# samivout/clair-torch

Measured on AMD Instinct MI355X. Metric: MPix/s HDR-merged (+uncertainty) at N=32 4K RGB, higher is better.
Workload: dtype f32; 1 GPU; C2: 32-exposure 4096x4096x3 uint16 stack per GPU, merge+uncertainty (LINEAR ICRF 3x256, Gaussian weights, sigma: multiplier, float64 mean + float32 std out); global_image=4096x4096x3 in 1 row band(s)

## Files before the change

### clair_torch_amd/csrc/ct_merge.hip

```cpp
#include "ct_merge.hpp"
#include <type_traits>

#ifndef CT_MERGE_PART
#define CT_MERGE_PART 0
#endif

namespace ct {

template <typename T, int V, int INTERP, int WEIGHT, int STD, bool FOLD, int PF = 2, bool PIVOT = true>
__global__ __launch_bounds__(kBlock) void merge_kernel(const MergeArgs a)
{
    extern __shared__ __align__(16) char lds[];
    constexpr bool kInt = sizeof(T) != 4;
    constexpr bool kRanged = kInt;
    constexpr bool kHasStd = STD != CT_STD_NONE;
    constexpr bool kGauss = WEIGHT == CT_WEIGHT_GAUSS;
    constexpr int kEntry = lut_entry_bytes(INTERP);
    static_assert(!FOLD || kInt, "FOLD is for integer codes");
    using Moment = std::conditional_t<PIVOT, float, double>;
    const int C = a.channels, L = a.n_points, B = a.batch;
    const int lut_bytes = INTERP == CT_INTERP_NONE ? 0 : C * L * kEntry;
    float *inv_t = reinterpret_cast<float *>(lds + lut_bytes);
    float *cq = inv_t + B;
    const float top = INTERP == CT_INTERP_NONE ? 1.0f : (float)(L - 1);
// ... 368 lines not shown
        __builtin_amdgcn_make_buffer_rsrc(reinterpret_cast<void *>(base), 0, 0xffffffff, 0x00020000 );
    P out;
    if constexpr (sizeof(P) == 1) {
        const uint8_t v = __builtin_amdgcn_raw_buffer_load_b8(rsrc, offset, 0, CT_STACK_LOAD_AUX);
        __builtin_memcpy(&out, &v, sizeof(P));
    } else if constexpr (sizeof(P) == 2) {
        const uint16_t v = __builtin_amdgcn_raw_buffer_load_b16(rsrc, offset, 0, CT_STACK_LOAD_AUX);
        __builtin_memcpy(&out, &v, sizeof(P));
    } else if constexpr (sizeof(P) == 4) {
        const uint32_t v = __builtin_amdgcn_raw_buffer_load_b32(rsrc, offset, 0, CT_STACK_LOAD_AUX);
        __builtin_memcpy(&out, &v, sizeof(P));
    } else if constexpr (sizeof(P) == 8) {
        typedef uint32_t vec_t __attribute__((ext_vector_type(2)));
        const vec_t v = __builtin_amdgcn_raw_buffer_load_b64(rsrc, offset, 0, CT_STACK_LOAD_AUX);
        __builtin_memcpy(&out, &v, sizeof(P));
    } else {
        static_assert(sizeof(P) == 16, "packets are at most 16 bytes");
        typedef uint32_t vec_t __attribute__((ext_vector_type(4)));
        const vec_t v = __builtin_amdgcn_raw_buffer_load_b128(rsrc, offset, 0, CT_STACK_LOAD_AUX);
        __builtin_memcpy(&out, &v, sizeof(P));
    }
    return out;
}

#ifndef CT_PIVOT_TYPED_LOAD
#define CT_PIVOT_TYPED_LOAD 1
#endif
template <typename T, int V>
__device__ __forceinline__ Packet<float, V> load_codes_as_float(uint64_t base, uint32_t offset)
{
    Packet<float, V> out;
    load_codes_as_float<T, V, CT_STACK_LOAD_AUX>(base, offset, out.v);
    return out;
}


template <int N, int I = 0, typename F>
__device__ __forceinline__ void static_for(F &&f)
{
    if constexpr (I < N) {
        f(std::integral_constant<int, I>{});
        static_for<N, I + 1>(f);
    }
}

struct PivotArgs {
    uint32_t index_mul;
    float step;
    uint32_t n_tiles;
    int32_t probe;
    float index_rcp;
    float max_code;
    float tf_max;
    uint32_t n_entries;
    unsigned long long *retry_count;
    int32_t n_batches;
    int32_t fresh;
    int32_t batch_size[16];
    const void *batch_ptr[16];
    const float *std_ptr[16];
    int32_t rgb252;
    uint32_t stage_off;
};
constexpr int kMaxMultiBatches = 16;
constexpr int kPivotV = 4;

#ifndef CT_PIVOT_DEPTH
#define CT_PIVOT_DEPTH 2
#endif
constexpr int kPivotDepth = CT_PIVOT_DEPTH;
constexpr float kRoughLimit = 64.0f;

#ifndef CT_PIVOT_WEIGHT
#define CT_PIVOT_WEIGHT 0
#endif
#ifndef CT_PIVOT_WT_SHIFT
#define CT_PIVOT_WT_SHIFT 4
#endif

#ifndef CT_RGB252_WAVES
#define CT_RGB252_WAVES 6
#endif
#ifndef CT_PIVOT_KERNEL_ATTR
#define CT_PIVOT_KERNEL_ATTR __attribute__((amdgpu_waves_per_eu(FIRST && V <= 4 && STD != CT_STD_EXPLICIT ? (CT_PIVOT_TYPED_LOAD ? (RGB252 ? CT_RGB252_WAVES : 7) : 8) : 4, 8)))
#endif
template <typename T, int V, int INTERP, int WEIGHT, int STD, bool FIRST, bool CLAMP = false, bool MULTI = false, bool RGB252 = false>
__global__ __launch_bounds__(kBlock) CT_PIVOT_KERNEL_ATTR void merge_pivot_kernel(const MergeArgs a, const PivotArgs x)
{
    static_assert(!MULTI || (!FIRST && CT_PIVOT_TYPED_LOAD), "MULTI carries state and uses the typed loads");
    static_assert(!RGB252 || (V == 4 && FIRST && !MULTI && CT_PIVOT_TYPED_LOAD), "RGB252: single-batch packets of the typed-load kernel");
    extern __shared__ __align__(16) char lds[];
    static_assert(sizeof(T) != 4, "raw integer codes only");
    static_assert(CT_PIVOT_TYPED_LOAD || ((INTERP == CT_INTERP_LINEAR || INTERP == CT_INTERP_NONE) && !CLAMP), "raw-load build: whole-step LINEAR only");
    constexpr bool kLut = INTERP != CT_INTERP_NONE;
    constexpr bool kLookup = INTERP == CT_INTERP_LOOKUP;
    constexpr bool kCat = INTERP == CT_INTERP_CATMULL;
    constexpr bool kHasStd = STD != CT_STD_NONE;
    constexpr bool kGauss = WEIGHT == CT_WEIGHT_GAUSS;
    constexpr bool kTyped = CT_PIVOT_TYPED_LOAD;
    using CodePk = std::conditional_t<kTyped, Packet<float, V>, Packet<T, V>>;
    const int C = a.channels, L = a.n_points, B = a.batch;
    constexpr int kWV = (INTERP == CT_INTERP_LINEAR && kGauss && kTyped && sizeof(T) == 2 && V == 4) ? CT_PIVOT_WEIGHT : 0;
    constexpr int kEntryShift = (kWV == 2 || kCat) ? 4 : 3;
    const int E = kLut ? (int)x.n_entries : 0;
    const int lut_bytes = C * E * (1 << kEntryShift);
    float2 *expo = reinterpret_cast<float2 *>(lds + lut_bytes);
    [[maybe_unused]] const uint32_t wt_base = (uint32_t)lut_bytes + 8u * (uint32_t)B;
    const float kk = sqrtf(a.weight_scale * 1.4426950408889634f);
    const float dk_mul = kk * a.inv_max_code, dk_add = -0.5f * kk;
    const float K = -2.0f * a.weight_scale;
    const float max_code = kLut ? x.max_code : 1.0f;
    const float ce = kGauss ? max_code * kk / K : max_code;

    bool rough = false;
    if constexpr (kLookup) {
        const int total = C * E;
        for (int k = threadIdx.x; k < total; k += kBlock) {
            const int r = k / E, j = k - r * E;
            const int idx = (j + 1) >> 1;
            reinterpret_cast<float2 *>(lds)[k] = make_float2(a.lut[(size_t)r * L + (idx < L ? idx : L - 1)], 0.0f);
        }
    } else if constexpr (kCat) {
        const int total = C * L;
        const double st = (double)x.step;
        for (int k = threadIdx.x; k < total; k += kBlock) {
            const int r = k / L, i = k - r * L;
            const float *row = a.lut + (size_t)r * L;
            const double p0 = row[i > 0 ? i - 1 : 0], p1 = row[i], p2 = row[i + 1 < L ? i + 1 : L - 1], p3 = row[i + 2 < L ? i + 2 : L - 1];
            const double c1 = 0.5 * (p2 - p0), b1 = 0.5 * (2.0 * p0 - 5.0 * p1 + 4.0 * p2 - p3), a1 = 0.5 * (-p0 + 3.0 * p1 - 3.0 * p2 + p3);
            reinterpret_cast<float4 *>(lds)[k] = make_float4((float)p1, (float)(c1 / st), (float)(b1 / (st * st)), (float)(a1 / (st * st * st)));
        }
    } else if constexpr (kLut) {
        const int total = C * L;
        const double stepd = (double)x.max_code / (double)(L - 1);
        bool viol = false;
        for (int k = threadIdx.x; k < total; k += kBlock) {
            const int r = k / L, i = k - r * L;
            const float *row = a.lut + (size_t)r * L;
            const float g0 = row[i], g1 = row[i + 1 < L ? i + 1 : L - 1];
            const float slope = (g1 - g0) / x.step;
            const float A = (float)((double)g0 - (double)slope * ((double)i * stepd));
            viol |= !(fabsf(A) <= kRoughLimit * fmaxf(fmaxf(fabsf(g0), fabsf(g1)), 1e-30f));
        }
        rough = __syncthreads_or(viol);
        for (int k = threadIdx.x; k < total; k += kBlock) {
            const int r = k / L, i = k - r * L;
            const float *row = a.lut + (size_t)r * L;
            const float g0 = row[i], g1 = row[i + 1 < L ? i + 1 : L - 1];
            const float slope = (g1 - g0) / x.step;
            const float A = (float)((double)g0 - (double)slope * ((double)i * stepd));
            if constexpr (kWV == 2) {
                const double dki = (double)i * (double)x.step * (double)dk_mul + (double)dk_add;
                reinterpret_cast<float4 *>(lds)[k] =
                    make_float4(rough ? g0 : A, slope, (float)exp2(-dki * dki), (float)(-2.0 * dki * (double)dk_mul));
            } else {
                reinterpret_cast<float2 *>(lds)[k] = make_float2(rough ? g0 : A, slope);
            }
        }
    }
    if constexpr (kWV == 1) {
        constexpr int s = CT_PIVOT_WT_SHIFT, nW = 65536 >> s;
        for (int j = threadIdx.x; j < nW; j += kBlock) {
            const double c0 = (double)(j << s), c1 = (double)((j + 1) << s);
            const double d0 = c0 * (double)dk_mul + (double)dk_add, d1 = c1 * (double)dk_mul + (double)dk_add;
            const double w0 = exp2(-d0 * d0), w1 = exp2(-d1 * d1), ws = (w1 - w0) / (c1 - c0);
            *reinterpret_cast<float2 *>(lds + wt_base + 8u * (uint32_t)j) = make_float2((float)(w0 - ws * c0), (float)ws);
        }
    }
    for (int n = threadIdx.x; n < B; n += kBlock) {
        const float it = (float)(1.0 / a.exposure[n]);
        expo[n] = make_float2(it, ce * it);
    }
    __syncthreads();

    const bool finalize = a.flags & CT_MERGE_FINALIZE;
    const bool keep_state = a.mean_state != nullptr;
    const bool planar = a.tile.layout == CT_LAYOUT_NCHW;
    const bool planar_out = planar || (a.flags & CT_MERGE_OUT_AS_INPUT);
    float fsf = 1.0f;
    if constexpr (kGauss) fsf = K / kk;
    if constexpr (STD == CT_STD_CONSTANT) fsf *= a.std_value;
    if constexpr (STD == CT_STD_MULTIPLIER) fsf *= a.std_value * a.inv_max_code;
    const float sv2 = fsf * fsf;
    [[maybe_unused]] const uint32_t index_mul = x.index_mul & 0xffffffu;
    [[maybe_unused]] const float index_rcp = x.index_rcp;
    [[maybe_unused]] float floor_magic = kFloorMagic;
    asm volatile("" : "+v"(floor_magic));

    constexpr bool rgb252 = RGB252;
    for (uint32_t tile = blockIdx.x; tile < x.n_tiles; tile += gridDim.x) {
        const uint32_t vec = tile * (uint32_t)kBlock + threadIdx.x;
        if (vec * (uint32_t)V >= a.q_count) continue;
        const uint32_t q0 = a.q_begin + vec * (uint32_t)V;

        int row_off[V];
        if constexpr (kLut) {
            if (planar) {
                int ch = 0;
                for (int c = 1; c < C; ++c) ch += q0 >= (uint32_t)c * a.tile.plane_local ? 1 : 0;
                const uint32_t qg = q0 + (uint32_t)ch * a.tile.chan_skip + a.tile.base;
                uint32_t off = q0 - (uint32_t)ch * a.tile.plane_local;
                int r = C == 3 ? (int)(qg % 3u) : (int)(qg % (uint32_t)C);
                const int skip_mod = (int)(a.tile.chan_skip % (uint32_t)C);
#pragma unroll
                for (int e = 0; e < V; ++e) {
                    row_off[e] = (kLookup ? ch : r) * E * 8;
                    int inc = 1;
                    if (++off == a.tile.plane_local) {
                        off = 0;
                        ++ch;
                        inc += skip_mod;
                    }
                    r += inc;
                    r = r >= C ? r - C : r;
                }
            } else if (C == 3) {
                const uint32_t plane_g = a.tile.plane_local + a.tile.chan_skip;
#pragma unroll
                for (int e = 0; e < V; ++e) {
                    uint32_t c, pixel;
                    a.tile.interleaved3(q0 + e, c, pixel);
                    const uint32_t qg = c * plane_g + a.tile.base + pixel;
                    row_off[e] = (int)(kLookup ? c : qg % 3u) * E * 8;
                }
            } else {
#pragma unroll
                for (int e = 0; e < V; ++e) {
                    int ch;
                    uint32_t qg;
                    a.tile.locate(a.tile.planar_index(q0 + e), ch, qg);
                    row_off[e] = (kLookup ? ch : (int)(qg % (uint32_t)C)) * E * 8;
                }
            }
        } else {
#pragma unroll
            for (int e = 0; e < V; ++e) row_off[e] = 0;
        }
        [[maybe_unused]] uint32_t rowc[V];
        if constexpr (kTyped && kLut) {
#pragma unroll
            for (int e = 0; e < V; ++e) rowc[e] = lds_row_constant<kEntryShift>(row_off[e] << (kEntryShift - 3));
        }

        const uint32_t voff = q0 * (uint32_t)sizeof(T), svoff = q0 * 4u;
        auto planar_of = [&](uint32_t m) -> uint32_t {
            if (planar_out) return m;
            if (C == 3) {
                uint32_t c, pixel;
                a.tile.interleaved3(m, c, pixel);
                return c * a.tile.plane_local + pixel;
            }
            return a.tile.planar_index(m);
        };

        constexpr int VS = FIRST ? 1 : V;
        float p[V], WA[VS], varA[VS];
        double meanA[VS];
        [[maybe_unused]] auto probe_pivot = [&](uint64_t stack_base) {
            const Packet<float, V> pk = load_codes_as_float<T, V>(
                stack_base + (uint64_t)((int64_t)x.probe * a.image_stride * (int64_t)sizeof(T)), voff);
            const float itp = expo[x.probe].x;
            float tf[V];
            if constexpr (kLut) floor_index_bits<V>(pk.v, index_rcp, floor_magic, tf);
            if constexpr (kLut && CLAMP) {
#pragma unroll
                for (int e = 0; e < V; ++e) tf[e] = fminf(tf[e], x.tf_max);
            }
#pragma unroll
            for (int e = 0; e < V; ++e) {
                const float px = pk.v[e];
                float lin = px * a.inv_max_code;
                if constexpr (kCat) {
                    const float4 g = *reinterpret_cast<const float4 *>(lds + lds_entry_address<kEntryShift>(tf[e], rowc[e]));
                    float o = __builtin_fmaf(tf[e] - floor_magic, -x.step, px);
                    if constexpr (CLAMP) o = px > x.max_code ? 0.0f : o;
                    lin = __builtin_fmaf(__builtin_fmaf(__builtin_fmaf(g.w, o, g.z), o, g.y), o, g.x);
                } else if constexpr (kLut) {
                    const float2 g = *reinterpret_cast<const float2 *>(lds + lds_entry_address<kEntryShift>(tf[e], rowc[e]));
                    lin = __builtin_fmaf(g.y, rough ? __builtin_fmaf(tf[e] - floor_magic, -x.step, px) : px, g.x);
                }
                p[e] = lin * itp;
            }
        };
        if constexpr (FIRST && kTyped) {
            probe_pivot(reinterpret_cast<uint64_t>(a.stack));
        } else if constexpr (FIRST) {
            const Packet<T, V> pk = load_buffer<Packet<T, V>>(
                reinterpret_cast<uint64_t>(a.stack) + (uint64_t)((int64_t)x.probe * a.image_stride * (int64_t)sizeof(T)), voff);
            const float itp = expo[x.probe].x;
            static_for<V>([&](auto ec) {
                constexpr int e = decltype(ec)::value;
                float lin = code_to_float<T, V, e>(pk) * a.inv_max_code;
                if constexpr (kLut) {
                    const uint32_t i0 = code_to_interval<T, V, e>(pk, index_mul);
                    const float2 g = *reinterpret_cast<const float2 *>(lds + (row_off[e] + (int)(i0 << 3)));
                    const float px = code_to_float<T, V, e>(pk);
                    lin = __builtin_fmaf(g.y, rough ? __builtin_fmaf((float)i0, -x.step, px) : px, g.x);
                }
                p[e] = lin * itp;
            });
        } else {
            bool fresh = false;
            if constexpr (MULTI) fresh = x.fresh != 0;
            if (fresh) {
                if constexpr (MULTI) {
#pragma unroll
                    for (int e = 0; e < V; ++e) {
                        meanA[e] = 0.0;
                        WA[e] = 0.0f;
                        varA[e] = 0.0f;
                    }
                    probe_pivot(reinterpret_cast<uint64_t>(x.batch_ptr[0]));
                }
            } else {
#pragma unroll
                for (int e = 0; e < V; ++e) {
                    const uint32_t q = planar_of(q0 + e);
                    meanA[e] = a.mean_state[q];
                    WA[e] = a.sumw_state[q];
                    if constexpr (kHasStd) varA[e] = a.var_state[q];
                    p[e] = (float)meanA[e];
                }
            }
        }

        double mean_o[V];
        float var_o[V], Wt_o[V];
        const int n_batches = MULTI ? x.n_batches : 1;
        int n0 = 0;
        for (int bi = 0; bi < n_batches; ++bi) {
        const int Bb = MULTI ? x.batch_size[bi] : B;
        const uint64_t batch_base = MULTI ? reinterpret_cast<uint64_t>(x.batch_ptr[bi]) : reinterpret_cast<uint64_t>(a.stack);
        [[maybe_unused]] const uint64_t batch_std_base = MULTI ? reinterpret_cast<uint64_t>(x.std_ptr[bi]) : reinterpret_cast<uint64_t>(a.std_stack);
        for (int pass = 0;; ++pass) {
            float W[V], Swy[V], Saa[V], Sac[V], Scc[V];
#pragma unroll
            for (int e = 0; e < V; ++e) W[e] = Swy[e] = Saa[e] = Sac[e] = Scc[e] = 0.0f;

            auto run_batch = [&](auto rough_c, auto moments_c) {
            constexpr bool kRough = decltype(rough_c)::value;
            constexpr bool kMoments = decltype(moments_c)::value;
            auto reduce = [&](const CodePk &pk, const Packet<float, V> &sp, uint32_t expo_adr) {
                const float2 ex = *reinterpret_cast<const float2 *>(lds + expo_adr);
                const float it = ex.x, cqn = ex.y;
                float pxv[V], ga[V], gs[V];
                [[maybe_unused]] float pxl[V];
                [[maybe_unused]] float dkv[V], wv[V];
                [[maybe_unused]] float tf[V], tw[V], gw[V], gd[V];
                if constexpr (kTyped) {
#pragma unroll
                    for (int e = 0; e < V; ++e) pxv[e] = pk.v[e];
                    if constexpr (kLut && kWV == 1)
                        floor_index_bits2<V>(pxv, index_rcp, 1.0f / (float)(1 << CT_PIVOT_WT_SHIFT), floor_magic, tf, tw);
                    else if constexpr (kLut)
                        floor_index_bits<V>(pxv, index_rcp, floor_magic, tf);
                    if constexpr (kLut && CLAMP) {
#pragma unroll
                        for (int e = 0; e < V; ++e) tf[e] = fminf(tf[e], x.tf_max);
                    }
                }
                static_for<V>([&](auto ec) {
                    constexpr int e = decltype(ec)::value;
                    if constexpr (kTyped) {
                        if constexpr (kLut && kWV == 2) {
                            float4 g = *reinterpret_cast<const float4 *>(lds + lds_entry_address<4>(tf[e], rowc[e]));
                            asm volatile("" : "+v"(g.x), "+v"(g.y), "+v"(g.z), "+v"(g.w));
                            ga[e] = g.x;
                            gs[e] = g.y;
                            gw[e] = g.z;
                            gd[e] = g.w;
                            pxl[e] = __builtin_fmaf(tf[e] - floor_magic, -x.step, pxv[e]);
                        } else if constexpr (kCat) {
                            const float4 g = *reinterpret_cast<const float4 *>(lds + lds_entry_address<4>(tf[e], rowc[e]));
                            float o = __builtin_fmaf(tf[e] - floor_magic, -x.step, pxv[e]);
                            [[maybe_unused]] bool above = false;
                            if constexpr (CLAMP) {
                                above = pxv[e] > x.max_code;
                                o = above ? 0.0f : o;
                            }
                            ga[e] = __builtin_fmaf(__builtin_fmaf(__builtin_fmaf(g.w, o, g.z), o, g.y), o, g.x);
                            gs[e] = 0.0f;
                            if constexpr (kHasStd) {
                                gs[e] = __builtin_fmaf(__builtin_fmaf(3.0f * g.w, o, g.z + g.z), o, g.y);
                                if constexpr (CLAMP) gs[e] = above ? 0.0f : gs[e];
                            }
                        } else if constexpr (kLut) {
                            const float2 g = *reinterpret_cast<const float2 *>(lds + lds_entry_address(tf[e], rowc[e]));
                            ga[e] = g.x;
                            gs[e] = g.y;
                            if constexpr (kRough) pxl[e] = __builtin_fmaf(tf[e] - floor_magic, -x.step, pxv[e]);
                            if constexpr (kWV == 1) {
                                const float2 wt = *reinterpret_cast<const float2 *>(
                                    lds + lds_entry_address(tw[e], wt_base - (kFloorMagicBits << 3)));
                                gw[e] = wt.x;
                                gd[e] = wt.y;
                            }
                        }
                    } else {
                    pxv[e] = code_to_float<T, V, e>(pk);
                    if constexpr (kLut) {
                        const uint32_t i0 = code_to_interval<T, V, e>(pk, index_mul);
                        const float2 g = *reinterpret_cast<const float2 *>(lds + (row_off[e] + (int)(i0 << 3)));
                        ga[e] = g.x;
                        gs[e] = g.y;
                        if constexpr (kRough) pxl[e] = __builtin_fmaf((float)i0, -x.step, pxv[e]);
                    }
                    }
                    if constexpr (kGauss) {
                        dkv[e] = __builtin_fmaf(pxv[e], dk_mul, dk_add);
                        if constexpr (kWV == 0) wv[e] = __builtin_amdgcn_exp2f(-dkv[e] * dkv[e]);
                    }
                });
                if constexpr (kWV == 1) {
#pragma unroll
                    for (int e = 0; e < V; ++e) wv[e] = __builtin_fmaf(gd[e], pxv[e], gw[e]);
                }
                if constexpr (kWV == 2) {
                    const float m2 = dk_mul * dk_mul;
#pragma unroll
                    for (int e = 0; e < V; ++e) {
                        const float v = pxl[e] * __builtin_fmaf(pxl[e], -m2, gd[e]);
                        float q = __builtin_fmaf(v, 0.009618129107628477f, 0.05550410866482158f);
                        q = __builtin_fmaf(q, v, 0.2402265069591007f);
                        q = __builtin_fmaf(q, v, 0.6931471805599453f);
                        q = __builtin_fmaf(q, v, 1.0f);
                        wv[e] = gw[e] * q;
                    }
                }
                if constexpr (kGauss && kWV == 0) {
#pragma unroll
                    for (int e = 0; e < V; ++e) asm volatile("" : "+v"(wv[e]));
                }
#pragma unroll
                for (int e = 0; e < V; ++e) {
                    const float px = pxv[e];
                    const float lin = (kLookup || kCat) ? ga[e] : kLut ? __builtin_fmaf(gs[e], kRough ? pxl[e] : px, ga[e]) : px * a.inv_max_code;
                    const float yd = __builtin_fmaf(lin, it, -p[e]);
                    if constexpr (kGauss) {
                        const float dk = dkv[e], w = wv[e];
                        W[e] += w;
                        Swy[e] = __builtin_fmaf(w, yd, Swy[e]);
                        if constexpr (kHasStd && kMoments) {
                            float wu = w;
                            if constexpr (STD == CT_STD_MULTIPLIER) wu = w * px;
                            if constexpr (STD == CT_STD_EXPLICIT) wu = w * sp.v[e];
                            const float av = dk * wu;
                            float cv;
                            if constexpr (kLookup) {
                                cv = av * yd;
                            } else {
                                const float ev = kLut ? (wu * gs[e]) * cqn : wu * cqn;
                                cv = __builtin_fmaf(av, yd, ev);
                            }
                            Saa[e] = __builtin_fmaf(av, av, Saa[e]);
                            Sac[e] = __builtin_fmaf(av, cv, Sac[e]);
                            Scc[e] = __builtin_fmaf(cv, cv, Scc[e]);
                        }
                    } else {
                        Swy[e] += yd;
                        if constexpr (kHasStd) {
                            float ev = kLut ? gs[e] * cqn : cqn;
                            if constexpr (STD == CT_STD_MULTIPLIER) ev *= px;
                            if constexpr (STD == CT_STD_EXPLICIT) ev *= sp.v[e];
                            Scc[e] = __builtin_fmaf(ev, ev, Scc[e]);
                        }
                    }
                }
            };

            auto fetch = [&](int n, CodePk &pk, Packet<float, V> &sp) {
                const int nn = n < Bb ? n : Bb - 1;
                uint64_t base = batch_base + (uint64_t)((int64_t)nn * a.image_stride * (int64_t)sizeof(T));
                asm volatile("" : "+s"(base));
                if constexpr (kTyped)
                    pk = load_codes_as_float<T, V>(base, voff);
                else
                    pk = load_buffer<Packet<T, V>>(base, voff);
                if constexpr (STD == CT_STD_EXPLICIT) {
                    uint64_t sbase = batch_std_base + (uint64_t)((int64_t)nn * a.image_stride * 4);
                    asm volatile("" : "+s"(sbase));
                    sp = load_buffer<Packet<float, V>>(sbase, svoff);
                }
            };
            constexpr int kRing = kPivotDepth + 1;
            CodePk ring[kRing];
            Packet<float, V> sring[STD == CT_STD_EXPLICIT ? kRing : 1];
            static_for<kPivotDepth>([&](auto jc) {
                constexpr int j = decltype(jc)::value;
                fetch(j, ring[j], sring[STD == CT_STD_EXPLICIT ? j : 0]);
            });
            uint32_t expo_adr = (uint32_t)lut_bytes + 8u * (uint32_t)n0;
            for (int n = 0; n < Bb; n += kRing) {
                static_for<kRing>([&](auto jc) {
                    constexpr int j = decltype(jc)::value, slot = (j + kPivotDepth) % kRing;
                    fetch(n + j + kPivotDepth, ring[slot], sring[STD == CT_STD_EXPLICIT ? slot : 0]);
                    if (j == 0 || n + j < Bb) reduce(ring[j], sring[STD == CT_STD_EXPLICIT ? j : 0], expo_adr + 8u * j);
                });
                expo_adr += 8u * kRing;
            }
            };
            constexpr bool kMeanFirst = kLookup && kHasStd;
            if constexpr (kMeanFirst) {
                if (pass == 0)
                    run_batch(std::false_type{}, std::false_type{});
                else
                    run_batch(std::false_type{}, std::true_type{});
            } else {
                if (rough)
                    run_batch(std::true_type{}, std::true_type{});
                else
                    run_batch(std::false_type{}, std::true_type{});
            }

            bool bad[V];
            float mb_f[V];
#pragma unroll
            for (int e = 0; e < V; ++e) {
                const float Wb = kGauss ? W[e] : (float)Bb;
                const float Df = Wb + 1e-6f;
                const float r = __builtin_amdgcn_rcpf(Df);
                const float num = __builtin_fmaf(-p[e], 1e-6f, Swy[e]);
                float q = num * r;
                q = __builtin_fmaf(__builtin_fmaf(-q, Df, num), r, q);
                float Wt = Wb, frac = 1.0f, var = 0.0f, gam = 0.0f;
                bad[e] = false;
                if constexpr (FIRST) {
                    mean_o[e] = (double)p[e] + (double)q;
                } else {
                    Wt = WA[e] + Wb;
                    const float rw = __builtin_amdgcn_rcpf(Wt);
                    frac = WA[e] == 0.0f ? 1.0f : Wb * rw;
                    const double diff = ((double)p[e] - meanA[e]) + (double)q;
                    mean_o[e] = __builtin_fma((double)frac, diff, meanA[e]);
                    gam = ((WA[e] * rw) * rw) * (float)diff;
                    var = varA[e];
                }
                Wt_o[e] = Wt;
                mb_f[e] = p[e] + q;
                if constexpr (kHasStd) {
                    const float beta = frac * r;
                    const float kap = __builtin_fmaf(-beta, q, gam);
                    const float bk = beta * kap;
                    const float S = __builtin_fmaf(kap * kap, Saa[e], (beta * beta) * Scc[e]);
                    const float upd = __builtin_fmaf(bk + bk, Sac[e], S);
                    if constexpr (kGauss) bad[e] = upd * (0.5f * (kPivotCondLimit + 1.0f)) < S;
                    if constexpr (kMeanFirst) bad[e] = bad[e] || pass == 0;
                    var += fmaxf(upd, 0.0f) * sv2;
                }
                var_o[e] = var;
            }
            bool any_bad = false;
#pragma unroll
            for (int e = 0; e < V; ++e) any_bad |= bad[e];
            if (pass == 1 || !__any(any_bad)) break;
            if (x.retry_count && (threadIdx.x & 63) == 0) atomicAdd(x.retry_count, 1ull);
#pragma unroll
            for (int e = 0; e < V; ++e) p[e] = bad[e] ? mb_f[e] : p[e];
        }
        if constexpr (MULTI) {
#pragma unroll
            for (int e = 0; e < V; ++e) {
                meanA[e] = mean_o[e];
                WA[e] = Wt_o[e];
                varA[e] = var_o[e];
                p[e] = (float)mean_o[e];
            }
            n0 += Bb;
        }
        }

        if (keep_state) {
#pragma unroll
            for (int e = 0; e < V; ++e) {
                const uint32_t q = planar_of(q0 + e);
                a.mean_state[q] = mean_o[e];
                a.sumw_state[q] = Wt_o[e];
                if constexpr (kHasStd) a.var_state[q] = var_o[e];
            }
        }
        if (finalize && rgb252) {
            if constexpr (RGB252) {
                const uint32_t tile_first = tile * (uint32_t)(kBlock * V);
// ... 354 lines not shown
        }
    }
    if (q_vec) {
        a.q_begin = 0;
        a.q_count = q_vec;
        rc = dispatch_interp<T, V>(a, interp, weight_mode, std_mode, s, fold);
        if (rc != CT_OK) return rc;
    }
    if (q_vec < Q) {
        a.q_begin = q_vec;
        a.q_count = Q - q_vec;
        rc = dispatch_interp<T, 1>(a, interp, weight_mode, std_mode, s, fold);
    }
    return rc;
}

#endif

}

#if CT_MERGE_PART != 1

extern "C" int ct_norm_constants(float max_code, float *hi, float *lo);
extern "C" int ct_index_constants(float max_code, int n_points, float *hi, float *lo);
extern "C" int ct_pivot_index_constants(float max_code, int n_points, uint32_t *index_mul, float *step);
extern "C" int ct_pivot_floor_constants(float max_code, int n_points, float *rcp_step);

static unsigned long long *g_merge_retry_counter = nullptr;
extern "C" void ct_merge_set_retry_counter(unsigned long long *counter_dev) { g_merge_retry_counter = counter_dev; }

extern "C" int ct_pivot_interval_constants(float max_code, int n_points, int lookup, int dtype_max, float *scale);

static bool pivot_eligible(int32_t dtype, float max_code, int interp, int n_points, uint32_t flags, ct::PivotArgs *px,
                           bool *clamp = nullptr)
{
    if (dtype != CT_DTYPE_U8 && dtype != CT_DTYPE_U16) return false;
    const int dtype_max = dtype == CT_DTYPE_U8 ? 255 : 65535;
    if (flags & CT_MERGE_F64_MOMENTS) return false;
    if (!(max_code >= 1.0f) || max_code > (float)dtype_max || floorf(max_code) != max_code) return false;
    if (interp < CT_INTERP_LOOKUP || interp > CT_INTERP_NONE) return false;
    if (interp == CT_INTERP_CATMULL && !CT_PIVOT_TYPED_LOAD) return false;
    const bool need_clamp = interp != CT_INTERP_NONE && max_code < (float)dtype_max;
    if (clamp) *clamp = need_clamp;
    px->step = 1.0f;
    px->index_mul = 0;
    px->index_rcp = 1.0f;
    px->max_code = max_code;
    px->n_entries = 0;
    px->tf_max = ct::kFloorMagic;
    if (interp == CT_INTERP_NONE) return true;
    if (CT_PIVOT_TYPED_LOAD) {
        if (need_clamp && dtype == CT_DTYPE_U8) return false;
        const bool lookup = interp == CT_INTERP_LOOKUP;
        if (ct_pivot_interval_constants(max_code, n_points, lookup, dtype_max, &px->index_rcp) != CT_OK) return false;
        px->step = (float)((double)max_code / (double)(n_points - 1));
        px->n_entries = lookup ? 2u * (uint32_t)n_points : (uint32_t)n_points;
        px->tf_max = ct::kFloorMagic + (float)(lookup ? 2 * (n_points - 1) : n_points - 1);
        return true;
    }
    if (interp != CT_INTERP_LINEAR || need_clamp) return false;
    if (ct_pivot_index_constants(max_code, n_points, &px->index_mul, &px->step) != CT_OK) return false;
    if (dtype == CT_DTYPE_U8 && px->step != 1.0f) return false;
    if (dtype == CT_DTYPE_U16 && px->index_mul == 0) return false;
    px->n_entries = (uint32_t)n_points;
    return true;
}

static bool merge_uses_reference_order(int interp, int std_mode, uint32_t flags)
{
    if (flags & CT_MERGE_REFERENCE_ORDER) return true;
    return (interp == CT_INTERP_CATMULL || interp == CT_INTERP_LOOKUP) && std_mode != CT_STD_NONE &&
           !(flags & (CT_MERGE_CLOSED_FORM | CT_MERGE_F64_MOMENTS));
}

extern "C" const char *ct_hdr_merge_kernel_name(int32_t dtype, float max_code, int32_t interp, int32_t n_points,
                                                uint32_t flags)
{
    if (merge_uses_reference_order(interp, (flags & CT_MERGE_STD_HINT) ? CT_STD_CONSTANT : CT_STD_NONE, flags))
        return "ct::merge_reference_order_kernel (the reference's float32 autograd order, two passes, float64 exp and divisions)";
    ct::PivotArgs px{};
    if (pivot_eligible(dtype, max_code, interp, interp == CT_INTERP_NONE ? 2 : n_points, flags, &px))
        return (flags & CT_MERGE_FIRST_BATCH)
                   ? "ct::merge_pivot_kernel (float32 moments about a per-pixel pivot, persistent workgroups, 4 codes per "
                     "thread through typed buffer loads, 7 wavefronts per SIMD, first batch)"
                   : "ct::merge_pivot_kernel (float32 moments about the running mean, persistent workgroups, 4 codes per "
                     "thread, streaming state)";
    if (flags & CT_MERGE_F64_MOMENTS)
        return dtype == CT_DTYPE_F32 ? "ct::merge_kernel (float64 moments, float32 pixels, 4 per thread)"
                                     : "ct::merge_kernel (float64 moments, integer codes)";
    return dtype == CT_DTYPE_F32 ? "ct::merge_kernel (float32 moments about a per-pixel pivot, float32 pixels, 4 per thread)"
                                 : "ct::merge_kernel (float32 moments about a per-pixel pivot, integer codes through the float LUT coordinate)";
}

extern "C" int ct_hdr_merge_batch(const void *stack_dev, int32_t dtype, float max_code, int32_t batch,
                                  const ct_geometry *geom, const float *std_dev, int32_t std_mode, float std_value,
                                  const double *exposure_dev, const ct_icrf *icrf, int32_t weight_mode,
                                  double *mean_state_dev, float *sumw_state_dev, float *var_state_dev,
                                  void *mean_out_dev, float *std_out_dev, uint32_t flags, void *stream)
{
    using namespace ct;
    if (!stack_dev || !geom || !icrf || !exposure_dev || batch <= 0) return CT_ERR_INVALID_ARGUMENT;
    if (geom->channels <= 0 || geom->h_tile <= 0 || geom->width <= 0 || geom->h_global < geom->h_tile ||
        geom->row_offset < 0 || geom->row_offset + geom->h_tile > geom->h_global)
        return CT_ERR_INVALID_ARGUMENT;
    if (geom->layout < CT_LAYOUT_NCHW || geom->layout > CT_LAYOUT_NHWC_BGR) return CT_ERR_INVALID_ARGUMENT;
    const int interp = icrf->interp;
    if (interp < CT_INTERP_LOOKUP || interp > CT_INTERP_NONE) return CT_ERR_INVALID_ARGUMENT;
    if (interp != CT_INTERP_NONE && (!icrf->lut_dev || icrf->n_points < 2)) return CT_ERR_INVALID_ARGUMENT;
    if (std_mode < CT_STD_NONE || std_mode > CT_STD_EXPLICIT) return CT_ERR_INVALID_ARGUMENT;
    if (std_mode == CT_STD_EXPLICIT && !std_dev) return CT_ERR_INVALID_ARGUMENT;
    if (weight_mode != CT_WEIGHT_NONE && weight_mode != CT_WEIGHT_GAUSS) return CT_ERR_INVALID_ARGUMENT;
    if (std_mode != CT_STD_NONE && interp == CT_INTERP_LOOKUP && weight_mode == CT_WEIGHT_NONE)
        return CT_ERR_NO_GRADIENT_PATH;
    const bool first = flags & CT_MERGE_FIRST_BATCH, finalize = flags & CT_MERGE_FINALIZE;
    const bool has_state = mean_state_dev && sumw_state_dev && (std_mode == CT_STD_NONE || var_state_dev);
    if (!has_state && !(first && finalize)) return CT_ERR_INVALID_ARGUMENT;
    if (finalize && (!mean_out_dev || (std_mode != CT_STD_NONE && !std_out_dev))) return CT_ERR_INVALID_ARGUMENT;

    const int64_t plane_g = geom->h_global * geom->width, plane_l = geom->h_tile * geom->width;
    const int64_t Qg = plane_g * geom->channels, Ql = plane_l * geom->channels;
    if (Qg >= (int64_t)1 << 31) return CT_ERR_TOO_LARGE;
    if (geom->image_stride < Ql) return CT_ERR_INVALID_ARGUMENT;

    MergeArgs a{};
    a.stack = stack_dev;
    a.std_stack = std_mode == CT_STD_EXPLICIT ? std_dev : nullptr;
    a.exposure = exposure_dev;
    a.lut = icrf->lut_dev;
    a.mean_state = has_state ? mean_state_dev : nullptr;
    a.sumw_state = has_state ? sumw_state_dev : nullptr;
    a.var_state = has_state ? var_state_dev : nullptr;
    a.mean_out = mean_out_dev;
    a.std_out = std_out_dev;
    a.image_stride = geom->image_stride;
    a.tile.plane_local = (uint32_t)plane_l;
    a.tile.chan_skip = (uint32_t)(plane_g - plane_l);
    a.tile.base = (uint32_t)(geom->row_offset * geom->width);
    a.tile.layout = (uint32_t)geom->layout;
    a.tile.channels = (uint32_t)geom->channels;
    a.batch = batch;
    a.channels = geom->channels;
    a.n_points = interp == CT_INTERP_NONE ? 2 : icrf->n_points;
    a.std_value = std_value;
    a.weight_scale = 30.0f;
    a.inv_max_code = 1.0f;
    a.flags = flags;
    hipStream_t s = static_cast<hipStream_t>(stream);
    if (merge_uses_reference_order(interp, std_mode, flags)) {
        if (dtype != CT_DTYPE_F32 && ct_norm_constants(max_code, &a.norm.hi, &a.norm.lo) != CT_OK) return CT_ERR_UNSUPPORTED;
        return merge_reference_order(a, dtype, (uint32_t)Ql, interp, weight_mode, std_mode, s);
    }
    switch (dtype) {
        case CT_DTYPE_U8:
        case CT_DTYPE_U16: {
            if (ct_norm_constants(max_code, &a.norm.hi, &a.norm.lo) != CT_OK) return CT_ERR_UNSUPPORTED;
            const bool fold = ct_index_constants(max_code, a.n_points, &a.index.hi, &a.index.lo) == CT_OK;
            a.inv_max_code = (float)(1.0 / (double)max_code);
            PivotArgs px{};
            const PivotArgs *pivot = nullptr;
            bool clamp = false;
            if (pivot_eligible(dtype, max_code, interp, a.n_points, flags, &px, &clamp)) {
                px.probe = batch / 2;
                px.retry_count = g_merge_retry_counter;
                pivot = &px;
            }
            return dtype == CT_DTYPE_U8 ? merge_typed<uint8_t>(a, (uint32_t)Ql, interp, weight_mode, std_mode, s, fold, pivot, clamp)
                                        : merge_typed<uint16_t>(a, (uint32_t)Ql, interp, weight_mode, std_mode, s, fold, pivot, clamp);
// ... 148 lines not shown
```

Measured before the change: 20020 MPix/s.

## Seed pivot from first pipelined load via rotated exposure order; split guarded tail

```diff
diff --git a/clair_torch_amd/csrc/ct_merge.hip b/clair_torch_amd/csrc/ct_merge.hip
--- a/clair_torch_amd/csrc/ct_merge.hip
+++ b/clair_torch_amd/csrc/ct_merge.hip
@@ -474,7 +474,7 @@
 #define CT_RGB252_WAVES 6
 #endif
 #ifndef CT_PIVOT_KERNEL_ATTR
-#define CT_PIVOT_KERNEL_ATTR __attribute__((amdgpu_waves_per_eu(FIRST && V <= 4 && STD != CT_STD_EXPLICIT ? (CT_PIVOT_TYPED_LOAD ? (RGB252 ? CT_RGB252_WAVES : 7) : 8) : 4, 8)))
+#define CT_PIVOT_KERNEL_ATTR __attribute__((amdgpu_waves_per_eu(FIRST && V <= 4 && STD != CT_STD_EXPLICIT ? (CT_PIVOT_TYPED_LOAD ? (RGB252 ? CT_RGB252_WAVES : 6) : 8) : 4, 8)))
 #endif
 template <typename T, int V, int INTERP, int WEIGHT, int STD, bool FIRST, bool CLAMP = false, bool MULTI = false, bool RGB252 = false>
 __global__ __launch_bounds__(kBlock) CT_PIVOT_KERNEL_ATTR void merge_pivot_kernel(const MergeArgs a, const PivotArgs x)
@@ -559,9 +559,15 @@
             *reinterpret_cast<float2 *>(lds + wt_base + 8u * (uint32_t)j) = make_float2((float)(w0 - ws * c0), (float)ws);
         }
     }
-    for (int n = threadIdx.x; n < B; n += kBlock) {
-        const float it = (float)(1.0 / a.exposure[n]);
-        expo[n] = make_float2(it, ce * it);
+    {
+        const int B0 = MULTI ? x.batch_size[0] : B;
+        const bool rotated = FIRST || (MULTI && x.fresh != 0);
+        for (int n = threadIdx.x; n < B; n += kBlock) {
+            int src = n;
+            if (rotated && n < B0) src = n + x.probe < B0 ? n + x.probe : n + x.probe - B0;
+            const float it = (float)(1.0 / a.exposure[src]);
+            expo[n] = make_float2(it, ce * it);
+        }
     }
     __syncthreads();
 
@@ -648,52 +654,9 @@
         constexpr int VS = FIRST ? 1 : V;
         float p[V], WA[VS], varA[VS];
         double meanA[VS];
-        [[maybe_unused]] auto probe_pivot = [&](uint64_t stack_base) {
-            const Packet<float, V> pk = load_codes_as_float<T, V>(
-                stack_base + (uint64_t)((int64_t)x.probe * a.image_stride * (int64_t)sizeof(T)), voff);
-            const float itp = expo[x.probe].x;
-            float tf[V];
-            if constexpr (kLut) floor_index_bits<V>(pk.v, index_rcp, floor_magic, tf);
-            if constexpr (kLut && CLAMP) {
-#pragma unroll
-                for (int e = 0; e < V; ++e) tf[e] = fminf(tf[e], x.tf_max);
-            }
-#pragma unroll
-            for (int e = 0; e < V; ++e) {
-                const float px = pk.v[e];
-                float lin = px * a.inv_max_code;
-                if constexpr (kCat) {
-                    const float4 g = *reinterpret_cast<const float4 *>(lds + lds_entry_address<kEntryShift>(tf[e], rowc[e]));
-                    float o = __builtin_fmaf(tf[e] - floor_magic, -x.step, px);
-                    if constexpr (CLAMP) o = px > x.max_code ? 0.0f : o;
-                    lin = __builtin_fmaf(__builtin_fmaf(__builtin_fmaf(g.w, o, g.z), o, g.y), o, g.x);
-                } else if constexpr (kLut) {
-                    const float2 g = *reinterpret_cast<const float2 *>(lds + lds_entry_address<kEntryShift>(tf[e], rowc[e]));
-                    lin = __builtin_fmaf(g.y, rough ? __builtin_fmaf(tf[e] - floor_magic, -x.step, px) : px, g.x);
-                }
-                p[e] = lin * itp;
-            }
-        };
-        if constexpr (FIRST && kTyped) {
-            probe_pivot(reinterpret_cast<uint64_t>(a.stack));
-        } else if constexpr (FIRST) {
-            const Packet<T, V> pk = load_buffer<Packet<T, V>>(
-                reinterpret_cast<uint64_t>(a.stack) + (uint64_t)((int64_t)x.probe * a.image_stride * (int64_t)sizeof(T)), voff);
-            const float itp = expo[x.probe].x;
-            static_for<V>([&](auto ec) {
-                constexpr int e = decltype(ec)::value;
-                float lin = code_to_float<T, V, e>(pk) * a.inv_max_code;
-                if constexpr (kLut) {
-                    const uint32_t i0 = code_to_interval<T, V, e>(pk, index_mul);
-                    const float2 g = *reinterpret_cast<const float2 *>(lds + (row_off[e] + (int)(i0 << 3)));
-                    const float px = code_to_float<T, V, e>(pk);
-                    lin = __builtin_fmaf(g.y, rough ? __builtin_fmaf((float)i0, -x.step, px) : px, g.x);
-                }
-                p[e] = lin * itp;
-            });
-        } else {
-            bool fresh = false;
-            if constexpr (MULTI) fresh = x.fresh != 0;
+        bool fresh = FIRST;
+        if constexpr (MULTI) fresh = x.fresh != 0;
+        if constexpr (!FIRST) {
             if (fresh) {
                 if constexpr (MULTI) {
 #pragma unroll
@@ -702,7 +665,6 @@
                         WA[e] = 0.0f;
                         varA[e] = 0.0f;
                     }
-                    probe_pivot(reinterpret_cast<uint64_t>(x.batch_ptr[0]));
                 }
             } else {
 #pragma unroll
@@ -724,7 +686,10 @@
         const int Bb = MULTI ? x.batch_size[bi] : B;
         const uint64_t batch_base = MULTI ? reinterpret_cast<uint64_t>(x.batch_ptr[bi]) : reinterpret_cast<uint64_t>(a.stack);
         [[maybe_unused]] const uint64_t batch_std_base = MULTI ? reinterpret_cast<uint64_t>(x.std_ptr[bi]) : reinterpret_cast<uint64_t>(a.std_stack);
+        const bool seeded = fresh && bi == 0;
+        const int rot = seeded ? x.probe : 0;
         for (int pass = 0;; ++pass) {
+            const bool seed = seeded && pass == 0;
             float W[V], Swy[V], Saa[V], Sac[V], Scc[V];
 #pragma unroll
             for (int e = 0; e < V; ++e) W[e] = Swy[e] = Saa[e] = Sac[e] = Scc[e] = 0.0f;
@@ -860,8 +825,8 @@
                 }
             };
 
-            auto fetch = [&](int n, CodePk &pk, Packet<float, V> &sp) {
-                const int nn = n < Bb ? n : Bb - 1;
+            auto fetch = [&](int k, CodePk &pk, Packet<float, V> &sp) {
+                const int nn = k + rot < Bb ? k + rot : k + rot - Bb;
                 uint64_t base = batch_base + (uint64_t)((int64_t)nn * a.image_stride * (int64_t)sizeof(T));
                 asm volatile("" : "+s"(base));
                 if constexpr (kTyped)
@@ -874,22 +839,64 @@
                     sp = load_buffer<Packet<float, V>>(sbase, svoff);
                 }
             };
+            auto seed_pivot = [&](const CodePk &pk, float itp) {
+                if constexpr (kTyped) {
+                    float tf[V];
+                    if constexpr (kLut) floor_index_bits<V>(pk.v, index_rcp, floor_magic, tf);
+                    if constexpr (kLut && CLAMP) {
+#pragma unroll
+                        for (int e = 0; e < V; ++e) tf[e] = fminf(tf[e], x.tf_max);
+                    }
+#pragma unroll
+                    for (int e = 0; e < V; ++e) {
+                        const float px = pk.v[e];
+                        float lin = px * a.inv_max_code;
+                        if constexpr (kCat) {
+                            const float4 g = *reinterpret_cast<const float4 *>(lds + lds_entry_address<kEntryShift>(tf[e], rowc[e]));
+                            float o = __builtin_fmaf(tf[e] - floor_magic, -x.step, px);
+                            if constexpr (CLAMP) o = px > x.max_code ? 0.0f : o;
+                            lin = __builtin_fmaf(__builtin_fmaf(__builtin_fmaf(g.w, o, g.z), o, g.y), o, g.x);
+                        } else if constexpr (kLut) {
+                            const float2 g = *reinterpret_cast<const float2 *>(lds + lds_entry_address<kEntryShift>(tf[e], rowc[e]));
+                            lin = __builtin_fmaf(g.y, kRough ? __builtin_fmaf(tf[e] - floor_magic, -x.step, px) : px, g.x);
+                        }
+                        p[e] = lin * itp;
+                    }
+                } else {
+                    static_for<V>([&](auto ec) {
+                        constexpr int e = decltype(ec)::value;
+                        float lin = code_to_float<T, V, e>(pk) * a.inv_max_code;
+                        if constexpr (kLut) {
+                            const uint32_t i0 = code_to_interval<T, V, e>(pk, index_mul);
+                            const float2 g = *reinterpret_cast<const float2 *>(lds + (row_off[e] + (int)(i0 << 3)));
+                            const float px = code_to_float<T, V, e>(pk);
+                            lin = __builtin_fmaf(g.y, kRough ? __builtin_fmaf((float)i0, -x.step, px) : px, g.x);
+                        }
+                        p[e] = lin * itp;
+                    });
+                }
+            };
             constexpr int kRing = kPivotDepth + 1;
             CodePk ring[kRing];
             Packet<float, V> sring[STD == CT_STD_EXPLICIT ? kRing : 1];
             static_for<kPivotDepth>([&](auto jc) {
                 constexpr int j = decltype(jc)::value;
-                fetch(j, ring[j], sring[STD == CT_STD_EXPLICIT ? j : 0]);
+                if (j < Bb) fetch(j, ring[j], sring[STD == CT_STD_EXPLICIT ? j : 0]);
             });
             uint32_t expo_adr = (uint32_t)lut_bytes + 8u * (uint32_t)n0;
-            for (int n = 0; n < Bb; n += kRing) {
+            if (seed) seed_pivot(ring[0], reinterpret_cast<const float2 *>(lds + expo_adr)->x);
+            auto trip = [&](int n, auto guard_c) {
+                constexpr bool kGuard = decltype(guard_c)::value;
                 static_for<kRing>([&](auto jc) {
                     constexpr int j = decltype(jc)::value, slot = (j + kPivotDepth) % kRing;
-                    fetch(n + j + kPivotDepth, ring[slot], sring[STD == CT_STD_EXPLICIT ? slot : 0]);
-                    if (j == 0 || n + j < Bb) reduce(ring[j], sring[STD == CT_STD_EXPLICIT ? j : 0], expo_adr + 8u * j);
+                    if (!kGuard || n + j + kPivotDepth < Bb) fetch(n + j + kPivotDepth, ring[slot], sring[STD == CT_STD_EXPLICIT ? slot : 0]);
+                    if (!kGuard || j == 0 || n + j < Bb) reduce(ring[j], sring[STD == CT_STD_EXPLICIT ? j : 0], expo_adr + 8u * j);
                 });
                 expo_adr += 8u * kRing;
-            }
+            };
+            int n = 0;
+            for (; n + (kRing - 1) + kPivotDepth < Bb; n += kRing) trip(n, std::false_type{});
+            for (; n < Bb; n += kRing) trip(n, std::true_type{});
             };
             constexpr bool kMeanFirst = kLookup && kHasStd;
             if constexpr (kMeanFirst) {
@@ -1410,7 +1417,7 @@
     if (pivot_eligible(dtype, max_code, interp, interp == CT_INTERP_NONE ? 2 : n_points, flags, &px))
         return (flags & CT_MERGE_FIRST_BATCH)
                    ? "ct::merge_pivot_kernel (float32 moments about a per-pixel pivot, persistent workgroups, 4 codes per "
-                     "thread through typed buffer loads, 7 wavefronts per SIMD, first batch)"
+                     "thread through typed buffer loads, 6 wavefronts per SIMD, first batch)"
                    : "ct::merge_pivot_kernel (float32 moments about the running mean, persistent workgroups, 4 codes per "
                      "thread, streaming state)";
     if (flags & CT_MERGE_F64_MOMENTS)
```

After: 20080 MPix/s (median of 6 runs). Within noise of the previous version (+0.3%).

## Rotate exposure order so the pivot probe reuses the first streamed frame

Applied to the files above, without the earlier changes.

```diff
diff --git a/clair_torch_amd/csrc/ct_merge.hip b/clair_torch_amd/csrc/ct_merge.hip
--- a/clair_torch_amd/csrc/ct_merge.hip
+++ b/clair_torch_amd/csrc/ct_merge.hip
@@ -559,8 +559,19 @@
             *reinterpret_cast<float2 *>(lds + wt_base + 8u * (uint32_t)j) = make_float2((float)(w0 - ws * c0), (float)ws);
         }
     }
+    int rot0 = 0, B0 = B;
+    if constexpr (FIRST) rot0 = x.probe;
+    if constexpr (MULTI) {
+        B0 = x.batch_size[0];
+        rot0 = x.fresh ? x.probe : 0;
+    }
     for (int n = threadIdx.x; n < B; n += kBlock) {
-        const float it = (float)(1.0 / a.exposure[n]);
+        int src = n;
+        if (n < B0) {
+            src = n + rot0;
+            src -= src >= B0 ? B0 : 0;
+        }
+        const float it = (float)(1.0 / a.exposure[src]);
         expo[n] = make_float2(it, ce * it);
     }
     __syncthreads();
@@ -648,50 +659,45 @@
         constexpr int VS = FIRST ? 1 : V;
         float p[V], WA[VS], varA[VS];
         double meanA[VS];
-        [[maybe_unused]] auto probe_pivot = [&](uint64_t stack_base) {
-            const Packet<float, V> pk = load_codes_as_float<T, V>(
-                stack_base + (uint64_t)((int64_t)x.probe * a.image_stride * (int64_t)sizeof(T)), voff);
-            const float itp = expo[x.probe].x;
-            float tf[V];
-            if constexpr (kLut) floor_index_bits<V>(pk.v, index_rcp, floor_magic, tf);
-            if constexpr (kLut && CLAMP) {
-#pragma unroll
-                for (int e = 0; e < V; ++e) tf[e] = fminf(tf[e], x.tf_max);
-            }
-#pragma unroll
-            for (int e = 0; e < V; ++e) {
-                const float px = pk.v[e];
-                float lin = px * a.inv_max_code;
-                if constexpr (kCat) {
-                    const float4 g = *reinterpret_cast<const float4 *>(lds + lds_entry_address<kEntryShift>(tf[e], rowc[e]));
-                    float o = __builtin_fmaf(tf[e] - floor_magic, -x.step, px);
-                    if constexpr (CLAMP) o = px > x.max_code ? 0.0f : o;
-                    lin = __builtin_fmaf(__builtin_fmaf(__builtin_fmaf(g.w, o, g.z), o, g.y), o, g.x);
-                } else if constexpr (kLut) {
-                    const float2 g = *reinterpret_cast<const float2 *>(lds + lds_entry_address<kEntryShift>(tf[e], rowc[e]));
-                    lin = __builtin_fmaf(g.y, rough ? __builtin_fmaf(tf[e] - floor_magic, -x.step, px) : px, g.x);
-                }
-                p[e] = lin * itp;
+        [[maybe_unused]] auto seed_pivot = [&](const CodePk &pk, uint32_t expo_adr) {
+            const float itp = reinterpret_cast<const float2 *>(lds + expo_adr)->x;
+            if constexpr (kTyped) {
+                float tf[V];
+                if constexpr (kLut) floor_index_bits<V>(pk.v, index_rcp, floor_magic, tf);
+                if constexpr (kLut && CLAMP) {
+#pragma unroll
+                    for (int e = 0; e < V; ++e) tf[e] = fminf(tf[e], x.tf_max);
+                }
+#pragma unroll
+                for (int e = 0; e < V; ++e) {
+                    const float px = pk.v[e];
+                    float lin = px * a.inv_max_code;
+                    if constexpr (kCat) {
+                        const float4 g = *reinterpret_cast<const float4 *>(lds + lds_entry_address<kEntryShift>(tf[e], rowc[e]));
+                        float o = __builtin_fmaf(tf[e] - floor_magic, -x.step, px);
+                        if constexpr (CLAMP) o = px > x.max_code ? 0.0f : o;
+                        lin = __builtin_fmaf(__builtin_fmaf(__builtin_fmaf(g.w, o, g.z), o, g.y), o, g.x);
+                    } else if constexpr (kLut) {
+                        const float2 g = *reinterpret_cast<const float2 *>(lds + lds_entry_address<kEntryShift>(tf[e], rowc[e]));
+                        lin = __builtin_fmaf(g.y, rough ? __builtin_fmaf(tf[e] - floor_magic, -x.step, px) : px, g.x);
+                    }
+                    p[e] = lin * itp;
+                }
+            } else {
+                static_for<V>([&](auto ec) {
+                    constexpr int e = decltype(ec)::value;
+                    float lin = code_to_float<T, V, e>(pk) * a.inv_max_code;
+                    if constexpr (kLut) {
+                        const uint32_t i0 = code_to_interval<T, V, e>(pk, index_mul);
+                        const float2 g = *reinterpret_cast<const float2 *>(lds + (row_off[e] + (int)(i0 << 3)));
+                        const float px = code_to_float<T, V, e>(pk);
+                        lin = __builtin_fmaf(g.y, rough ? __builtin_fmaf((float)i0, -x.step, px) : px, g.x);
+                    }
+                    p[e] = lin * itp;
+                });
             }
         };
-        if constexpr (FIRST && kTyped) {
-            probe_pivot(reinterpret_cast<uint64_t>(a.stack));
-        } else if constexpr (FIRST) {
-            const Packet<T, V> pk = load_buffer<Packet<T, V>>(
-                reinterpret_cast<uint64_t>(a.stack) + (uint64_t)((int64_t)x.probe * a.image_stride * (int64_t)sizeof(T)), voff);
-            const float itp = expo[x.probe].x;
-            static_for<V>([&](auto ec) {
-                constexpr int e = decltype(ec)::value;
-                float lin = code_to_float<T, V, e>(pk) * a.inv_max_code;
-                if constexpr (kLut) {
-                    const uint32_t i0 = code_to_interval<T, V, e>(pk, index_mul);
-                    const float2 g = *reinterpret_cast<const float2 *>(lds + (row_off[e] + (int)(i0 << 3)));
-                    const float px = code_to_float<T, V, e>(pk);
-                    lin = __builtin_fmaf(g.y, rough ? __builtin_fmaf((float)i0, -x.step, px) : px, g.x);
-                }
-                p[e] = lin * itp;
-            });
-        } else {
+        if constexpr (!FIRST) {
             bool fresh = false;
             if constexpr (MULTI) fresh = x.fresh != 0;
             if (fresh) {
@@ -702,7 +708,6 @@
                         WA[e] = 0.0f;
                         varA[e] = 0.0f;
                     }
-                    probe_pivot(reinterpret_cast<uint64_t>(x.batch_ptr[0]));
                 }
             } else {
 #pragma unroll
@@ -724,6 +729,8 @@
         const int Bb = MULTI ? x.batch_size[bi] : B;
         const uint64_t batch_base = MULTI ? reinterpret_cast<uint64_t>(x.batch_ptr[bi]) : reinterpret_cast<uint64_t>(a.stack);
         [[maybe_unused]] const uint64_t batch_std_base = MULTI ? reinterpret_cast<uint64_t>(x.std_ptr[bi]) : reinterpret_cast<uint64_t>(a.std_stack);
+        const int rot = bi == 0 ? rot0 : 0;
+        const bool seeded = FIRST || (MULTI && x.fresh && bi == 0);
         for (int pass = 0;; ++pass) {
             float W[V], Swy[V], Saa[V], Sac[V], Scc[V];
 #pragma unroll
@@ -861,7 +868,9 @@
             };
 
             auto fetch = [&](int n, CodePk &pk, Packet<float, V> &sp) {
-                const int nn = n < Bb ? n : Bb - 1;
+                int nn = n < Bb ? n : Bb - 1;
+                nn += rot;
+                nn -= nn >= Bb ? Bb : 0;
                 uint64_t base = batch_base + (uint64_t)((int64_t)nn * a.image_stride * (int64_t)sizeof(T));
                 asm volatile("" : "+s"(base));
                 if constexpr (kTyped)
@@ -882,14 +891,19 @@
                 fetch(j, ring[j], sring[STD == CT_STD_EXPLICIT ? j : 0]);
             });
             uint32_t expo_adr = (uint32_t)lut_bytes + 8u * (uint32_t)n0;
-            for (int n = 0; n < Bb; n += kRing) {
+            auto trip = [&](int n, bool seed) {
                 static_for<kRing>([&](auto jc) {
                     constexpr int j = decltype(jc)::value, slot = (j + kPivotDepth) % kRing;
                     fetch(n + j + kPivotDepth, ring[slot], sring[STD == CT_STD_EXPLICIT ? slot : 0]);
+                    if constexpr (j == 0) {
+                        if (seed) seed_pivot(ring[0], expo_adr);
+                    }
                     if (j == 0 || n + j < Bb) reduce(ring[j], sring[STD == CT_STD_EXPLICIT ? j : 0], expo_adr + 8u * j);
                 });
                 expo_adr += 8u * kRing;
-            }
+            };
+            trip(0, pass == 0 && seeded);
+            for (int n = kRing; n < Bb; n += kRing) trip(n, false);
             };
             constexpr bool kMeanFirst = kLookup && kHasStd;
             if constexpr (kMeanFirst) {
```

Result: slower. 18650 MPix/s before, 18210 MPix/s after, median of 2 (-2.4%).
